# iliasam/STM32F4_SDR_GPS

Hardware: AMD Instinct MI355X
Metric: acquisition hypotheses/sec (PRN x Doppler x phase) (higher is better)
Workload: dtype u1 (MX-FP4 operands, exact f32 accumulation)

## Files before the change

stm32f4_sdr_gps_amd/csrc/gpsx_mx_parts.hpp:

```cpp
#pragma once
#if !defined(GPSX_LAB) && defined(MX_VARIANT_B)
#error "variants of the matrix-core grid kernels for same-box A/B timing build with -DGPSX_LAB only: tools/build_variant.sh"
#endif
#include <cstdlib>

#include "gpsx_anchor_codes.hpp"
#include "gpsx_device.hpp"
#include "gpsx_fold_codes.hpp"
#include "gpsx_kernels.hpp"

namespace gpsx {

namespace {

typedef int v8i __attribute__((ext_vector_type(8)));
typedef int v4i __attribute__((ext_vector_type(4)));
typedef float v16f __attribute__((ext_vector_type(16)));

constexpr int kMxThreads = 512;
constexpr int kMxTiles = 4;
constexpr int kCopyDwords = 260;
constexpr int kVecDwords = 258;
constexpr int kPlaneWordsMx = 66;
constexpr u32 kScaleOne = 0x7F7F7F7Fu;
constexpr u32 kScaleA = 0x72727272u;
constexpr float kAccScale = 1.0f / 8192.0f;
constexpr float kUnscaleSq = 67108864.0f;
constexpr u32 kScaleEight = 0x82828282u;
constexpr u32 kScaleTwo = 0x80808080u;

struct MxShared {
  uint16_t x[1024];
  u32 d[2][514];
  u32 plane[2][16][kPlaneWordsMx];
  u32 base[2][kCopyDwords];
  u32 e8[2][2][8][kCopyDwords];
  u32 corr[2][2][2][128];
  v4i chips_a[16][2][32];
  u32 chip_t[1032];
  u32 ones[2];
  u32 t_lut[768];
  alignas(16) u32 part[8][32][2][32];
};

struct MxFold {
  u32 pair[2][2][1024];
  v4i lut[2][32];
};

__device__ __forceinline__ v8i widen(v4i x) { return v8i{x.x, x.y, x.z, x.w, 0, 0, 0, 0}; }

__device__ __forceinline__ u32 lds_byte(const u32 *words, int byte_index)
{
  return (words[byte_index >> 2] >> ((byte_index & 3) * 8)) & 0xFFu;
}

__device__ __forceinline__ u32 spread8(u32 x)
{
  u32 t = (x | (x << 12)) & 0x000F000Fu;
  t = (t | (t << 6)) & 0x03030303u;
  t = (t | (t << 3)) & 0x11111111u;
  return t;
}

__device__ __forceinline__ int wrap1023(int i)
{
  i = i >= 2 * kChips ? i - 2 * kChips : i;
  return i >= kChips ? i - kChips : i;
}

__device__ __forceinline__ u32 plane_bits9(const u32 *pl, int pos)
{
  return __builtin_amdgcn_alignbit(pl[(pos >> 5) + 1], pl[pos >> 5], (u32)(pos & 31)) & 0x1FFu;
}

struct MxCluster {
  int set, sd, dopp, search;
};
__device__ __forceinline__ MxCluster mx_decode_cluster(int cluster, int n_sets, int n_dopp)
{
  const int set = cluster % n_sets, sd = cluster / n_sets;
  return MxCluster{set, sd, sd % n_dopp, sd / n_dopp};
}
__device__ __forceinline__ u32 mx_step_word(int dopp, int if_hz, int dopp_min_hz, int dopp_step_hz)
{
  const float freq_hz = (float)(if_hz + dopp_min_hz + dopp * dopp_step_hz);
  return nco_step_per_word(freq_hz);
}
__device__ __forceinline__ void mx_load_chips_a(MxShared &sh, const u32 *__restrict__ mx_a, int set, int tid)
{
  const u32 *src_a = mx_a + (size_t)set * (16 * 2 * 32 * 4);
  u32 *dst_a = reinterpret_cast<u32 *>(&sh.chips_a[0][0][0]);
  for (int i = tid; i < 16 * 2 * 32 * 4; i += kMxThreads)
    dst_a[i] = src_a[i];
}
__device__ __forceinline__ void mx_load_tables(MxShared &sh, const u32 *__restrict__ mx_a, const u32 *__restrict__ mx_t, int set, int tid)
{
  mx_load_chips_a(sh, mx_a, set, tid);
  const u32 *src_t = mx_t + (size_t)set * 1032;
  for (int i = tid; i < 1032; i += kMxThreads)
    sh.chip_t[i] = src_t[i];
}

__device__ __forceinline__ void mx_load_block(MxShared &sh, const uint8_t *blk, int if_format, int tid)
{
  for (int i = tid; i < 1024; i += kMxThreads)
    sh.x[i] = i < kWords16 ? load_sign16(blk, i, if_format) : (uint16_t)0;
  if (tid < 2)
    sh.ones[tid] = 0;
}
template <bool WRAP_IN_PLACE = false>
__device__ __forceinline__ void mx_wipe_stream(MxShared &sh, u32 step_word, int tid, int lane)
{
  {
    const u32 *x32 = reinterpret_cast<const u32 *>(sh.x);
    u32 ones_i = 0, ones_q = 0;
    for (int w = tid; w < 514; w += kMxThreads) {
      u32 vi = 0, vq = 0;
      if (w < kWords32) {
        const u32 quad = (step_word * (u32)w) >> 30;
        vi = carrier_i(quad) ^ x32[w];
        vq = carrier_q(quad) ^ x32[w];
      }
      ones_i += __popc(vi);
      ones_q += __popc(vq);
      if (WRAP_IN_PLACE && w == 511) {
        vi = (carrier_i(0u) ^ x32[0]) << 16;
        vq = (carrier_q(0u) ^ x32[0]) << 16;
      }
      sh.d[0][w] = vi;
      sh.d[1][w] = vq;
    }
    ones_i = wave_sum_to_lane63(ones_i);
    ones_q = wave_sum_to_lane63(ones_q);
    if (lane == 63) {
      atomicAdd(&sh.ones[0], ones_i);
      atomicAdd(&sh.ones[1], ones_q);
    }
  }
  if constexpr (!WRAP_IN_PLACE) {
    __syncthreads();
    if (tid < 2)
      sh.d[tid][511] = sh.d[tid][0] << 16;
  }
}
// ... 8 lines not shown
  }
  return v;
}
__device__ void mx_wipe_block(MxShared &sh, u32 step_word, int tid, int lane)
{
  mx_wipe_stream(sh, step_word, tid, lane);
  __syncthreads();
  for (int m = tid; m < 2 * 32 * 16; m += kMxThreads) {
    const int t0 = m & 15, w = (m >> 4) & 31, iq = m >> 9;
    const u32 *src = &sh.d[iq][16 * w];
    u32 bits = 0;
#pragma unroll
    for (int k = 0; k < 16; k++) {
      const u32 sk = src[k];
      bits |= ((sk >> t0) & 1u) << (2 * k);
      bits |= ((sk >> (16 + t0)) & 1u) << (2 * k + 1);
    }
    sh.plane[iq][t0][w] = bits;
  }
  __syncthreads();
  for (int m = tid; m < 2 * 16 * (kPlaneWordsMx - 32); m += kMxThreads) {
    const int w = 32 + m % (kPlaneWordsMx - 32);
    const int r = m / (kPlaneWordsMx - 32);
    sh.plane[r >> 4][r & 15][w] = mx_plane_ext_word(sh.plane[r >> 4][r & 15], w);
  }
}

__device__ __forceinline__ u32 fp4_code(int v)
{
  const u32 m = (u32)(v < 0 ? -v : v);
  return ((0x0765420u >> (4u * (m > 5u ? 5u : m))) & 0xFu) | (v < 0 ? 8u : 0u);
}

__device__ void mx_fill_tables(MxShared &sh, int tid, int nthreads = kMxThreads)
{
  for (int w = tid; w < 512; w += nthreads) {
    const u32 cur = (u32)w & 0xFFu, nxt = ((u32)w >> 1) & 0xFFu;
    const u32 plus = spread8(nxt & ~cur), minus = spread8(cur & ~nxt);
    sh.t_lut[w] = (plus << 2) | (plus << 3) | (minus << 2);
  }
  for (int x = tid; x < 256; x += nthreads)
    sh.t_lut[512 + x] = (spread8((u32)x) << 1) | (spread8(~(u32)x & 0xFFu) * 0xAu);
}

__device__ void mx_vector_phase1(MxShared &sh, int pass, int buf, int tid)
{
  const int t0 = pass - 1;
  for (int m = tid; m < 2 * kVecDwords + 2 * 128; m += kMxThreads) {
    if (m < 2 * kVecDwords) {
      const int iq = m >= kVecDwords, dw = m - iq * kVecDwords;
      u32 packed = 0;
      if (pass < 2) {
        const u32 *dd = sh.d[iq];
#pragma unroll
        for (int e = 0; e < 8; e++) {
          const int k = wrap1023(8 * dw + e);
          const int pos = 16 * k;
          const u32 sum = pop16(__builtin_amdgcn_alignbit(dd[(pos >> 5) + 1], dd[pos >> 5], (u32)(pos & 31)));
          const u32 code = pass == 0 ? (0xFEC0u >> (4u * (sum & 3u))) & 0xFu : (0xEDCA0u >> (4u * (sum >> 2))) & 0xFu;
          packed |= code << (4 * e);
        }
      } else {
        const u32 w = plane_bits9(sh.plane[iq][pass - 2], 8 * dw);
        packed = sh.t_lut[w];
        if (dw == 127 && t0 >= 9) {
          const u32 cur = w & 0xFFu, nxt = (w >> 1) & 0xFFu;
          const int e5 = (int)((nxt >> 5) & 1u) - (int)((cur >> 5) & 1u), e6 = (int)((nxt >> 6) & 1u) - (int)((cur >> 6) & 1u);
// ... 31 lines not shown
{
  for (int m = tid; m < 2 * 256; m += kMxThreads) {
    const int iq = m >> 8, j = m & 255;
    const u32 lo = sh.base[iq][j], hi = sh.base[iq][j + 1];
#pragma unroll
    for (int c = 0; c < 8; c++)
      sh.e8[buf][iq][c][j] = c ? __builtin_amdgcn_alignbit(hi, lo, 4u * (u32)c) : lo;
  }
}

typedef __attribute__((address_space(3))) const u32 lds_cu32;

__device__ __forceinline__ lds_cu32 *lds_opaque(const u32 *p)
{
  u32 a = (u32)(size_t)(lds_cu32 *)p;
  asm volatile("" : "+v"(a));
  return (lds_cu32 *)(size_t)a;
}
__device__ __forceinline__ v4i lds_frag(lds_cu32 *w, int dw)
{
  return v4i{(int)w[dw], (int)w[dw + 1], (int)w[dw + 2], (int)w[dw + 3]};
}

__device__ __forceinline__ u32 mx_patch_wrap(u32 packed, u32 w9, bool patch)
{
  const u32 i5 = 1u + ((w9 >> 6) & 1u) - ((w9 >> 5) & 1u), i6 = 1u + ((w9 >> 7) & 1u) - ((w9 >> 6) & 1u);
  const u32 c5 = (0xDA2u >> (4u * i5)) & 0xFu;
  const u32 c6 = (0xA25u >> (4u * i6)) & 0xFu;
  const u32 patched = (packed & ~0x0FF00000u) | (c5 << 20) | (c6 << 24);
  return patch ? patched : packed;
}

template <bool FOLD = false>
__device__ __forceinline__ void mx_vector_build(MxShared &sh, int p_vec, int tid, MxFold *fold = nullptr)
{
  const int t0 = p_vec - 1, buf = p_vec & 1;
  const bool late = t0 >= 9;
  const int iq = tid >> 8, j = tid & 255, which = (tid >> 7) & 1, dwc = tid & 127;
  const u32 *pl = sh.plane[iq][p_vec - 2];
  const u32 x = __builtin_amdgcn_alignbit(pl[(j >> 2) + 1], pl[j >> 2], 8u * (u32)(j & 3));
  u32 cw = 0, v = 0;
  if constexpr (!FOLD) {
    const int pos = dwc ? 8 * dwc - 1 : 0;
    const u32 y = __builtin_amdgcn_alignbit(pl[(pos >> 5) + 1], pl[pos >> 5], (u32)(pos & 31));
    cw = (dwc ? y : y << 1) & 0x1FFu;
  }
  u32 lo = sh.t_lut[x & 0x1FFu], hi = sh.t_lut[(x >> 8) & 0x1FFu];
  if constexpr (!FOLD)
    v = sh.t_lut[which ? 512u + (cw & 0xFFu) : (late ? cw : 512u + (cw >> 1))];
  if (late) {
    lo = mx_patch_wrap(lo, x & 0x1FFu, j == 127);
    hi = mx_patch_wrap(hi, (x >> 8) & 0x1FFu, j == 126);
    if constexpr (!FOLD) {
      if (which == 0)
        v ^= (v & 0x44444444u) << 1;
      if (dwc == 0)
        v = (v & ~0xFu) | (which ? 0u : ((cw & 2u) ? 0x2u : 0xAu));
    }
  }
  if constexpr (!FOLD) {
    v &= dwc == 127 ? 0x0FFFFFFFu : 0xFFFFFFFFu;
    if ((which && !late) || t0 == 8)
      v = 0;
    sh.corr[buf][iq][which][dwc] = v;
  } else {
    const int pos = 4 * j + kChips - 2;
    const u32 z = __builtin_amdgcn_alignbit(pl[(pos >> 5) + 1], pl[pos >> 5], (u32)(pos & 31)) & 31u;
    v4i pr = fold->lut[late][z];
    if (late && j == 0) {
      pr.x = (int)(gpsx_fold_pair(true, 0, (int)(z & 1u), (int)((z >> 1) & 1u)) << kGpsxFoldShift);
      pr.y = (int)(gpsx_fold_pair(true, 1, (int)((z >> 1) & 1u), (int)((z >> 2) & 1u)) << kGpsxFoldShift);
    }
    *reinterpret_cast<v4i *>(&fold->pair[buf][iq][4 * j]) = pr;
  }
  u32 *dst = &sh.e8[buf][iq][0][j];
#pragma unroll
  for (int c = 0; c < 8; c++)
    dst[c * kCopyDwords] = c ? __builtin_amdgcn_alignbit(hi, lo, 4u * (u32)c) : lo;
}

struct MxFoldRegs {
  lds_cu32 *w;
  u32 mask, pi, pq;
};
template <int S, int NT, u32 SCALE_A = kScaleA, bool FOLD = false>
__device__ __forceinline__ void mx_pass_step(lds_cu32 *wi, lds_cu32 *wq, const v4i *ca, v4i (&a)[16], v4i &fi, v4i &fq,
                                             v16f (&acc)[2][NT], u32 scale_b, MxFoldRegs *fold = nullptr)
{
  constexpr int kSteps = 16 + NT - 1;
  constexpr bool more = S + 1 < kSteps;
  constexpr bool pair_next = FOLD && more && S + 1 >= 15, patched = FOLD && S >= 15;
  v4i fi_next = fi, fq_next = fq;
  u32 pi_next = 0, pq_next = 0;
  if constexpr (more) {
    fi_next = lds_frag(wi, 8 * (S + 1));
    fq_next = lds_frag(wq, 8 * (S + 1));
    if constexpr (S + 1 < 16)
      a[S + 1] = ca[(S + 1) * 64];
    if constexpr (pair_next) {
      pi_next = fold->w[64 * (S + 1 - 15)];
      pq_next = fold->w[64 * (S + 1 - 15) + 1024];
    }
  }
  constexpr int j_lo = S - 15 > 0 ? S - 15 : 0, j_hi = S < NT - 1 ? S : NT - 1;
#pragma unroll
  for (int j = j_lo + (patched ? 1 : 0); j <= j_hi; j++) {
    acc[0][j] = __builtin_amdgcn_mfma_scale_f32_32x32x64_f8f6f4(widen(a[S - j]), widen(fi), acc[0][j], 4, 4, 0, SCALE_A, 0, scale_b);
    acc[1][j] = __builtin_amdgcn_mfma_scale_f32_32x32x64_f8f6f4(widen(a[S - j]), widen(fq), acc[1][j], 4, 4, 0, SCALE_A, 0, scale_b);
  }
  if constexpr (patched) {
    fi.w = (int)((fold->mask & fold->pi) | (~fold->mask & (u32)fi.w));
    fq.w = (int)((fold->mask & fold->pq) | (~fold->mask & (u32)fq.w));
    acc[0][j_lo] = __builtin_amdgcn_mfma_scale_f32_32x32x64_f8f6f4(widen(a[15]), widen(fi), acc[0][j_lo], 4, 4, 0, SCALE_A, 0, scale_b);
    acc[1][j_lo] = __builtin_amdgcn_mfma_scale_f32_32x32x64_f8f6f4(widen(a[15]), widen(fq), acc[1][j_lo], 4, 4, 0, SCALE_A, 0, scale_b);
  }
  if constexpr (more) {
    __builtin_amdgcn_sched_group_barrier(0x100, (S + 1 < 16 ? 5 : 4) + (pair_next ? 2 : 0), 0);
    if constexpr (patched) {
      __builtin_amdgcn_sched_group_barrier(0x008, 2 * (j_hi - j_lo), 0);
      __builtin_amdgcn_sched_group_barrier(0x002, 2, 0);
      __builtin_amdgcn_sched_group_barrier(0x008, 2, 0);
    } else {
      __builtin_amdgcn_sched_group_barrier(0x008, 2 * (j_hi - j_lo + 1), 0);
    }
  }
  __builtin_amdgcn_sched_barrier(0);
  fi = fi_next;
  fq = fq_next;
  if constexpr (FOLD) {
    fold->pi = pi_next;
    fold->pq = pq_next;
  }
  if constexpr (more)
    mx_pass_step<S + 1, NT, SCALE_A, FOLD>(wi, wq, ca, a, fi, fq, acc, scale_b, fold);
}

template <int S, int NT>
__device__ __forceinline__ void mx_pass_step_inplace(lds_cu32 *wi, lds_cu32 *wq, const v4i *ca, v4i (&a)[16], v4i &fi, v4i &fq,
                                                     v16f (&acc)[2][NT], u32 scale_b)
{
  constexpr int kSteps = 16 + NT - 1;
  constexpr bool more = S + 1 < kSteps;
  if constexpr (more && S + 1 < 16)
    a[S + 1] = ca[(S + 1) * 64];
  constexpr int j_lo = S - 15 > 0 ? S - 15 : 0, j_hi = S < NT - 1 ? S : NT - 1;
#pragma unroll
  for (int j = j_lo; j <= j_hi; j++)
    acc[0][j] = __builtin_amdgcn_mfma_scale_f32_32x32x64_f8f6f4(widen(a[S - j]), widen(fi), acc[0][j], 4, 4, 0, kScaleA, 0, scale_b);
  if constexpr (more)
    fi = lds_frag(wi, 8 * (S + 1));
#pragma unroll
  for (int j = j_lo; j <= j_hi; j++)
    acc[1][j] = __builtin_amdgcn_mfma_scale_f32_32x32x64_f8f6f4(widen(a[S - j]), widen(fq), acc[1][j], 4, 4, 0, kScaleA, 0, scale_b);
  if constexpr (more)
    fq = lds_frag(wq, 8 * (S + 1));
  if constexpr (more) {
    if constexpr (S + 1 < 16)
      __builtin_amdgcn_sched_group_barrier(0x100, 1, 0);
    __builtin_amdgcn_sched_group_barrier(0x008, j_hi - j_lo + 1, 0);
    __builtin_amdgcn_sched_group_barrier(0x100, 2, 0);
    __builtin_amdgcn_sched_group_barrier(0x008, j_hi - j_lo + 1, 0);
    __builtin_amdgcn_sched_group_barrier(0x100, 2, 0);
  }
  __builtin_amdgcn_sched_barrier(0);
  if constexpr (more)
    mx_pass_step_inplace<S + 1, NT>(wi, wq, ca, a, fi, fq, acc, scale_b);
}

template <bool AHEAD, int NT, u32 SCALE_A = kScaleA, bool FOLD = false>
__device__ __forceinline__ void mx_pass(const MxShared &sh, int buf, int lane, int q0_tile, v16f (&acc)[2][NT],
                                        u32 scale_b, v4i a_corr, bool with_corr, const u32 *fold_pair = nullptr)
{
  static_assert(!FOLD || (AHEAD && NT == kMxTiles), "the fold is the single-block form's");
  const int n = lane & 31, h = lane >> 5;
  const u32 *e8 = &sh.e8[buf][0][0][0];
  lds_cu32 *wi = lds_opaque(e8 + (n & 7) * kCopyDwords + 4 * (q0_tile + h) + (n >> 3));
  lds_cu32 *wq = lds_opaque(e8 + (8 + (n & 7)) * kCopyDwords + 4 * (q0_tile + h) + (n >> 3));
  const v4i *ca = &sh.chips_a[0][h][n];
  v4i a[16];
  if constexpr (AHEAD) {
    v4i fi = lds_frag(wi, 0), fq = lds_frag(wq, 0);
    a[0] = ca[0];
    if constexpr (FOLD) {
      MxFoldRegs fold{lds_opaque(fold_pair + 32 * q0_tile + n), h && with_corr ? kGpsxFoldMask : 0u, 0u, 0u};
      mx_pass_step<0, NT, SCALE_A, true>(wi, wq, ca, a, fi, fq, acc, scale_b, &fold);
    } else {
      mx_pass_step<0, NT, SCALE_A>(wi, wq, ca, a, fi, fq, acc, scale_b);
    }
  } else {
    static_assert(SCALE_A == kScaleA, "the in-place walk is the sign-only grid's");
    v4i fi = lds_frag(wi, 0), fq = lds_frag(wq, 0);
    a[0] = ca[0];
    mx_pass_step_inplace<0, NT>(wi, wq, ca, a, fi, fq, acc, scale_b);
  }
  if (!FOLD && with_corr) {
    lds_cu32 *cw = lds_opaque(&sh.corr[buf][0][h][4 * q0_tile + (n >> 3)]);
#pragma unroll
    for (int j = 0; j < NT; j++) {
      const v4i gi = v4i{(int)(cw[8 * j] >> (4 * (n & 7))), 0, 0, 0};
      const v4i gq = v4i{(int)(cw[8 * j + 2 * 128] >> (4 * (n & 7))), 0, 0, 0};
      acc[0][j] = __builtin_amdgcn_mfma_scale_f32_32x32x64_f8f6f4(widen(a_corr), widen(gi), acc[0][j], 4, 4, 0, kScaleA, 0,
                                                                   kScaleOne);
      acc[1][j] = __builtin_amdgcn_mfma_scale_f32_32x32x64_f8f6f4(widen(a_corr), widen(gq), acc[1][j], 4, 4, 0, kScaleA, 0,
// ... 239 lines not shown
```

stm32f4_sdr_gps_amd/csrc/k_acq_mx.hip:

```cpp
#include "gpsx_mx_parts.hpp"

namespace gpsx {

__global__ void k_build_mx_tables(const u32 *__restrict__ chipbits, int n_slots, u32 *__restrict__ mx_a, u32 *__restrict__ mx_t)
{
  const int n_sets = (n_slots + 31) / 32;
  const int idx = blockIdx.x * blockDim.x + threadIdx.x;
  const int per_set = 16 * 2 * 32 * 4 + 1032;
  if (idx >= n_sets * per_set)
    return;
  const int set = idx / per_set, r = idx - set * per_set;
  if (r < 16 * 2 * 32 * 4) {
    const int dw = r & 3, p = (r >> 2) & 31, h = (r >> 7) & 1, kappa = r >> 8;
    const int slot = 32 * set + p;
    const u32 word = slot < n_slots ? chipbits[(size_t)slot * 32 + 2 * kappa + h] : 0u;
    mx_a[(size_t)set * (16 * 2 * 32 * 4) + r] = spread8((word >> (8 * dw)) & 0xFFu) << 1;
  } else {
    const int c = r - 16 * 2 * 32 * 4 - 1;
    u32 w = 0;
    if (c >= 0 && c < kChips)
      for (int p = 0; p < 32; p++) {
        const int slot = 32 * set + p;
        if (slot < n_slots)
          w |= ((chipbits[(size_t)slot * 32 + (c >> 5)] >> (c & 31)) & 1u) << p;
      }
    mx_t[(size_t)set * 1032 + (c + 1)] = w;
  }
}

void launch_build_mx_tables(hipStream_t s, const uint32_t *d_chipbits, int n_slots, uint32_t *d_mx_a, uint32_t *d_mx_t)
{
  const int n_sets = (n_slots + 31) / 32;
  const int n = n_sets * (16 * 2 * 32 * 4 + 1032);
  hipLaunchKernelGGL(k_build_mx_tables, dim3((n + 255) / 256), dim3(256), 0, s, d_chipbits, n_slots, d_mx_a, d_mx_t);
}

namespace {

constexpr int kMxNoSet = -1;
constexpr int kPasses = 17;
constexpr int kPassesAnchor = 16;
constexpr int kAnchorDwords = 392;

__device__ __forceinline__ void mx_planes_half(MxShared &sh, int t0_lo, int v, int lane)
{
  const int iq = v >> 1, t0_first = t0_lo + 4 * (v & 1);
  const int t0 = t0_first + (lane & 3), rot = lane >> 2;
#pragma unroll 1
  for (int it = 0; it < 2; it++) {
    const int w = rot + 16 * it;
    const u32 *src = &sh.d[iq][16 * w];
    u32 bits = 0;
#pragma unroll
    for (int k = 0; k < 16; k++) {
      const int kk = (k + rot) & 15;
      const u32 sk = src[kk];
      bits |= ((sk >> t0) & 1u) << (2 * kk);
      bits |= ((sk >> (16 + t0)) & 1u) << (2 * kk + 1);
    }
    sh.plane[iq][t0][w] = bits;
  }
  __builtin_amdgcn_fence(__ATOMIC_ACQ_REL, "wavefront");
  asm volatile("s_waitcnt lgkmcnt(0)" ::: "memory");
#pragma unroll 1
  for (int m = lane; m < 4 * (kPlaneWordsMx - 32); m += 64) {
    const int r = m / (kPlaneWordsMx - 32), w = 32 + m % (kPlaneWordsMx - 32);
    u32 *pl = sh.plane[iq][t0_first + r];
    pl[w] = mx_plane_ext_word(pl, w);
  }
}

__device__ __forceinline__ void mx_anchor_build(MxShared &sh, u32 *dst, int tid)
{
  const int iq = tid >> 8, j = tid & 255;
  const u32 *dd = sh.d[iq];
  u64 bits = 0;
#pragma unroll
  for (int e = 0; e < 8; e++) {
    const int pos = 16 * wrap1023(8 * j + e);
    const u32 sum = pop16(__builtin_amdgcn_alignbit(dd[(pos >> 5) + 1], dd[pos >> 5], (u32)(pos & 31)));
    bits |= (u64)gpsx_anchor_code((int)sum) << (6 * e);
  }
  const u32 lo = (u32)bits, hi = (u32)(bits >> 32);
  const u32 lo_pair = dpp<0xB1>(lo, lo);
  u32 *d3 = dst + iq * kAnchorDwords + 3 * (j >> 1);
  if (j & 1) {
    d3[2] = (lo >> 16) | (hi << 16);
  } else {
    d3[0] = lo;
    d3[1] = hi | (lo_pair << 16);
  }
}

struct AnchorRaw {
  u32 d[7];
};
__device__ __forceinline__ AnchorRaw mx_anchor_raw(lds_cu32 *w, int dw)
{
  AnchorRaw r;
#pragma unroll
  for (int i = 0; i < 7; i++)
    r.d[i] = w[dw + i];
  return r;
}
__device__ __forceinline__ v8i mx_anchor_frag(const AnchorRaw &r, u32 shift)
{
  v8i f = {0, 0, 0, 0, 0, 0, 0, 0};
#pragma unroll
  for (int i = 0; i < 6; i++)
    f[i] = (int)__builtin_amdgcn_alignbit(r.d[i + 1], r.d[i], shift);
  return f;
}
template <int S, int NT>
__device__ __forceinline__ void mx_anchor_step(lds_cu32 *wi, lds_cu32 *wq, const v4i *ca, v4i (&a)[16], v8i &fi, v8i &fq,
                                               v16f (&acc)[2][NT], u32 shift)
{
  constexpr int kSteps = 16 + NT - 1;
  constexpr bool more = S + 1 < kSteps;
  AnchorRaw ri, rq;
  if constexpr (more) {
    ri = mx_anchor_raw(wi, 12 * (S + 1));
    rq = mx_anchor_raw(wq, 12 * (S + 1));
    if constexpr (S + 1 < 16)
      a[S + 1] = ca[(S + 1) * 64];
  }
  constexpr int j_lo = S - 15 > 0 ? S - 15 : 0, j_hi = S < NT - 1 ? S : NT - 1;
#pragma unroll
  for (int j = j_lo; j <= j_hi; j++) {
    acc[0][j] = __builtin_amdgcn_mfma_scale_f32_32x32x64_f8f6f4(widen(a[S - j]), fi, acc[0][j], 4, 3, 0, kScaleA, 0, kScaleTwo);
    acc[1][j] = __builtin_amdgcn_mfma_scale_f32_32x32x64_f8f6f4(widen(a[S - j]), fq, acc[1][j], 4, 3, 0, kScaleA, 0, kScaleTwo);
  }
  if constexpr (more) {
    __builtin_amdgcn_sched_group_barrier(0x100, S + 1 < 16 ? 9 : 8, 0);
    __builtin_amdgcn_sched_group_barrier(0x008, 2 * (j_hi - j_lo + 1), 0);
  }
  __builtin_amdgcn_sched_barrier(0);
  if constexpr (more) {
    fi = mx_anchor_frag(ri, shift);
    fq = mx_anchor_frag(rq, shift);
    __builtin_amdgcn_sched_barrier(0);
    mx_anchor_step<S + 1, NT>(wi, wq, ca, a, fi, fq, acc, shift);
  }
}
template <int NT>
__device__ __forceinline__ void mx_anchor_pass(const MxShared &sh, const u32 *anchor, int lane, int q0_tile, v16f (&acc)[2][NT])
{
  const int n = lane & 31, h = lane >> 5;
  const u32 shift = (u32)(6 * n) & 31u;
  lds_cu32 *wi = lds_opaque(anchor + 6 * (q0_tile + h) + ((6 * n) >> 5));
  lds_cu32 *wq = lds_opaque(anchor + kAnchorDwords + 6 * (q0_tile + h) + ((6 * n) >> 5));
  const v4i *ca = &sh.chips_a[0][h][n];
  v4i a[16];
  v8i fi = mx_anchor_frag(mx_anchor_raw(wi, 0), shift), fq = mx_anchor_frag(mx_anchor_raw(wq, 0), shift);
  a[0] = ca[0];
  mx_anchor_step<0, NT>(wi, wq, ca, a, fi, fq, acc, shift);
}

__device__ __forceinline__ void mx_vector_build_direct(MxShared &sh, int which, int t0s, u32 *e8_dst, int tid)
{
  const int iq = tid >> 8, j = tid & 255;
  const u32 *dd = sh.d[iq];
  u32 w2[2] = {0, 0};
#pragma unroll
  for (int e = 0; e < 16; e++) {
    const int k = wrap1023(8 * j + e);
    const int pos = 16 * k + t0s;
    const u32 sum = pop16(__builtin_amdgcn_alignbit(dd[(pos >> 5) + 1], dd[pos >> 5], (u32)(pos & 31)));
    const u32 code = which == 0 ? (0xFEC0u >> (4u * (sum & 3u))) & 0xFu : (0xEDCA0u >> (4u * (sum >> 2))) & 0xFu;
    w2[e >> 3] |= code << (4 * (e & 7));
  }
  u32 *dst = e8_dst + (iq * 8) * kCopyDwords + j;
#pragma unroll
  for (int c = 0; c < 8; c++)
    dst[c * kCopyDwords] = c ? __builtin_amdgcn_alignbit(w2[1], w2[0], 4u * (u32)c) : w2[0];
}

__device__ __forceinline__ void mx_direct_terms(const MxShared &sh, int lane, int q0_tile, v16f (&acc)[2][kMxTiles], int t0s,
                                                int win_start, int win_stop)
// ... 252 lines not shown
  if (SEARCH && !DIRECT) {
#pragma unroll
    for (int r = 0; r < 16; r++) {
      const int p_off = ((r & 3) + 8 * (r >> 2)) * 64;
      atomicMax(slot + p_off, best[DIRECT ? 0 : r]);
      atomicAdd(slot + p_off + 32, total[DIRECT ? 0 : r]);
    }
  }
}

__device__ __forceinline__ void mx_epilogue_store(int lane, int q0_tile, int t0, const v16f (&acc)[2][kMxTiles], u32 group_mask,
                                                  uint16_t *__restrict__ plane0, size_t prn_stride, int slot0, int n_prn)
{
  const int n = lane & 31, h = lane >> 5;
#pragma unroll
  for (int j = 0; j < kMxTiles; j++) {
    const int q = 32 * (q0_tile + 2 * j) + n;
    uint16_t *v = plane0 + (size_t)t0 * 1024 + (size_t)(q & 3) * 256 + (size_t)(q >> 2);
#pragma unroll
    for (int g = 0; g < 4; g++) {
#pragma unroll
      for (int rr = 0; rr < 4; rr++) {
        const int r = 4 * g + rr;
        const int p = (r & 3) + 8 * (r >> 2) + 4 * h;
        const u32 val = mag8_f32(acc[0][j][r], acc[1][j][r]);
        if (((group_mask >> g) & 1u) && slot0 + p < n_prn)
          v[(size_t)p * prn_stride] = (uint16_t)val;
      }
      __builtin_amdgcn_sched_barrier(0);
    }
  }
}

struct MxSingleShared {
  MxShared mx;
  MxFold fold;
};
__device__ __forceinline__ void mx_fill_fold_lut(MxFold &fold, int t)
{
  if (t < 64) {
    const int late = t >> 5, z = t & 31;
    v4i e;
#pragma unroll
    for (int i = 0; i < 4; i++)
      e[i] = (int)(gpsx_fold_pair(late != 0, 2, (z >> i) & 1, (z >> (i + 1)) & 1) << kGpsxFoldShift);
    fold.lut[late][z] = e;
  }
}

__device__ __forceinline__ void mx_single(MxShared &sh, MxFold &fold, const AcqParams &prm, int cluster_lo,
                                          const uint8_t *__restrict__ if_blocks, const u32 *__restrict__ mx_a,
                                          const u32 *__restrict__ mx_t, gpsx_peak_t *__restrict__ peaks)
{
  const int tid = threadIdx.x;
  const int lane = tid & 63, wave = __builtin_amdgcn_readfirstlane(tid >> 6);
  const int role = wave >> 2;
  const int q0_tile = 8 * (wave >> 1) + (wave & 1);

  const int n_sets = (prm.n_groups + 3) / 4;
  const MxCluster c = mx_decode_cluster(cluster_lo + (int)blockIdx.x, n_sets, prm.n_dopp);
  const int set = c.set, sd = c.sd, dopp = c.dopp, search = c.search;
  u32 group_mask = 0;
#pragma unroll
  for (int g = 0; g < 4; g++) {
    const int group = 4 * set + g;
    const int unit = sd * prm.n_groups + group;
    if (group < prm.n_groups && unit >= prm.unit_lo && unit < prm.unit_hi)
      group_mask |= 1u << g;
  }
  group_mask = (u32)__builtin_amdgcn_readfirstlane((int)group_mask);
  if (group_mask == 0)
    return;
  const u32 step_word = mx_step_word(dopp, prm.if_hz, prm.dopp_min_hz, prm.dopp_step_hz);

  if (set != kMxNoSet) {
    mx_load_tables(sh, mx_a, mx_t, set, tid);
  }
  for (int i = tid; i < 8 * 32 * 2 * 32 / 4; i += kMxThreads)
    reinterpret_cast<uint4 *>(&sh.part[0][0][0][0])[i] = make_uint4(0, 0, 0, 0);
  const size_t block_bytes = prm.if_format == GPSX_IF_2BIT_SM ? GPSX_BYTES_PER_MS_2BIT : kBytes;
  const uint8_t *block0 = if_blocks + (size_t)(search * prm.search_stride_blocks) * block_bytes;
  mx_load_block(sh, block0, prm.if_format, tid);

  __syncthreads();
  u32 kq[kMxTiles];
#pragma unroll
  for (int j = 0; j < kMxTiles; j++) {
    kq[j] = (u32)(2047 - 2 * (32 * (q0_tile + 2 * j) + (lane & 31)));
    asm volatile("" : "+v"(kq[j]));
  }
  const int n_pass = kPassesAnchor;
#pragma unroll 1
  for (int once = 0; once < 1; once++) {
    mx_wipe_stream<true>(sh, step_word, tid, lane);
    __syncthreads();
    mx_anchor_build(sh, &sh.e8[0][0][0][0], tid);

    v16f acc[2][kMxTiles];
    if (role == 0)
      mx_init_acc(sh.ones, lane, q0_tile, acc, prm.win_start, prm.win_stop, kGpsxAnchorPassBias);

    auto opaque = [](int v) {
      asm volatile("" : "+v"(v));
      return v;
    };
    __syncthreads();
    if (role) {
      mx_planes_half(sh, 0, wave & 3, opaque(lane));
      mx_fill_tables(sh, opaque(tid) & 255, 256);
      mx_fill_fold_lut(fold, opaque(tid) & 255);
      mx_planes_half(sh, 8, wave & 3, opaque(lane));
      mx_init_acc(sh.ones, opaque(lane), q0_tile, acc, prm.win_start, prm.win_stop, kGpsxAnchorPassBias);
    }
    mx_anchor_pass(sh, &sh.e8[0][0][0][0], lane, q0_tile, acc);
    if (!role)
      mx_epilogue_single(sh, lane, kq, 0, acc);
    __syncthreads();
    mx_vector_build<true>(sh, 2, opaque(tid), &fold);
#pragma unroll 1
    for (int hs = 2; hs <= 2 * n_pass; hs++) {
      if ((hs & 1) == 0) {
        __syncthreads();
        const int p_vec = (hs >> 1) + 1;
        if (p_vec < n_pass)
          mx_vector_build<true>(sh, p_vec + 1, tid, &fold);
      }
      const int x = hs - role;
      const bool active = x >= 0 && x < 2 * n_pass;
      const int p = (x >> 1) + 1;
      if (active && (x & 1) == 0) {
        mx_pass<true, kMxTiles, kScaleA, true>(sh, p & 1, lane, q0_tile, acc, p == 1 ? kScaleEight : kScaleOne, v4i{0, 0, 0, 0},
                                               p >= 2 && p != 9, &fold.pair[p & 1][0][0]);
        if (p == 9)
          mx_half_switch(sh, lane, q0_tile, acc, prm.win_start, prm.win_stop);
      }
      if (active && (x & 1) && p >= 1)
        mx_epilogue_single(sh, lane, kq, p - 1, acc);
    }
  }
  __syncthreads();
  {
    const int which = tid >> 8, p = (tid >> 3) & 31, b = tid & 7;
    const int slot = 32 * set + p;
    const u32 *row = sh.part[b][p][which];
    u32 vals[32];
#pragma unroll
    for (int l = 0; l < 32; l++)
      vals[l] = row[(l + tid) & 31];
    u32 k = 0, t = 0;
#pragma unroll
    for (int l = 0; l < 32; l++) {
      k = vals[l] > k ? vals[l] : k;
      t += vals[l];
    }
    if (((group_mask >> (p >> 3)) & 1u) && slot < prm.n_prn && b < prm.n_bits) {
      const size_t idx = ((size_t)(search * prm.n_prn + slot) * prm.n_dopp + dopp) * prm.n_bits + b;
      uint2 *pk = reinterpret_cast<uint2 *>(&peaks[idx]);
      if (which == 0) {
        const u32 max_val = k >> 11;
        pk[0] = make_uint2(max_val, max_val ? 2047u - (k & 2047u) : 0u);
      } else {
        pk[1] = make_uint2(t, t / (2u * kChips));
      }
    }
    if (prm.keys && which == 0) {
      unsigned long long key = 0;
      if (b < prm.n_bits) {
        const u32 max_val = k >> 11, phase = max_val ? 2047u - (k & 2047u) : 0u;
        key = ((unsigned long long)max_val << 14) | (unsigned long long)(16383u - (8u * phase + (u32)b));
      }
      key = mx_max8_u64(key);
      if (b == 0 && ((group_mask >> (p >> 3)) & 1u) && slot < prm.n_prn)
        prm.keys[(size_t)(search * prm.n_prn + slot) * prm.n_dopp + dopp] = (int64_t)key;
    }
  }
}

template <int MODE>
__device__ __forceinline__ void mx_unit(MxShared &sh, const AcqParams &prm, int cluster_lo,
                                        const uint8_t *__restrict__ if_blocks, const u32 *__restrict__ mx_a,
                                        const u32 *__restrict__ mx_t, gpsx_peak_t *__restrict__ peaks, u32 *__restrict__ energy,
                                        u32 *__restrict__ flags)
{
  constexpr bool MULTI = MODE == kMxWalk || MODE == kMxWalk16, STORE = MODE == kMxStore, S16 = MODE == kMxWalk16;
  constexpr bool SPLIT = MODE == kMxSplit;
  typedef SumRecT<S16> SumRec;
  const int wg = (int)blockIdx.x;
// ... 184 lines not shown
        if (which == 0)
          atomicMax(&energy[idx], k);
        else
          atomicAdd(&energy[n_planes + idx], t);
      } else if (which == 0) {
        const u32 max_val = k >> 11;
        pk[0] = make_uint2(max_val, max_val ? 2047u - (k & 2047u) : 0u);
      } else {
        pk[1] = make_uint2(t, t / (2u * kChips));
      }
    }
    if constexpr (!SPLIT) {
      if (prm.keys && which == 0) {
        unsigned long long key = 0;
        if (b < prm.n_bits) {
          const u32 max_val = k >> 11, phase = max_val ? 2047u - (k & 2047u) : 0u;
          key = ((unsigned long long)max_val << 14) | (unsigned long long)(16383u - (8u * phase + (u32)b));
        }
        key = mx_max8_u64(key);
        if (b == 0 && ((group_mask >> (p >> 3)) & 1u) && slot < prm.n_prn)
          prm.keys[(size_t)(search * prm.n_prn + slot) * prm.n_dopp + dopp] = (int64_t)key;
      }
    }
  }
}

}

template <int MODE>
__global__ __launch_bounds__(kMxThreads, 1) void k_acq_mx(GPSX_K_ACQ_MX_PARAMS)
{
  if constexpr (MODE == kMxSingle) {
    __shared__ MxSingleShared sh;
    mx_single(sh.mx, sh.fold, prm, cluster_lo, if_blocks, mx_a, mx_t, peaks);
  } else {
    __shared__ MxShared sh;
    mx_unit<MODE>(sh, prm, cluster_lo, if_blocks, mx_a, mx_t, peaks, energy, flags);
  }
}

void launch_acq_mx(hipStream_t s, const AcqPlan &p, const AcqParams &prm, const uint8_t *d_if, const uint32_t *d_mx_a,
                   const uint32_t *d_mx_t, uint32_t *d_planes, uint32_t *d_energy)
{
  if (p.c_hi <= p.c_lo)
    return;
  const dim3 grid((unsigned)p.grid), block(kMxThreads);
  gpsx_peak_t *d_peaks = prm.peaks;
  switch (p.form) {
  case AcqForm::kMxStore:
    hipLaunchKernelGGL(k_acq_mx<kMxStore>, grid, block, 0, s, prm, p.c_lo, d_if, d_mx_a, d_mx_t, d_peaks, d_energy, (u32 *)nullptr);
    launch_acq_vals_search(s, prm, reinterpret_cast<const uint16_t *>(d_energy), d_peaks, p.n_peaks);
    break;
  case AcqForm::kMxWalk: {
    u32 *d_flags = d_energy + acq_mx_energy_bytes(p.grid) / sizeof(u32) - p.grid;
    (void)hipMemsetAsync(d_flags - kMxZeroRecBytes / sizeof(u32), 0, kMxZeroRecBytes, s);
    hipLaunchKernelGGL(k_acq_mx<kMxWalk16>, grid, block, 0, s, prm, p.c_lo, d_if, d_mx_a, d_mx_t, d_peaks, d_energy, d_flags);
    if (p.walk24)
      hipLaunchKernelGGL(k_acq_mx<kMxWalk>, grid, block, 0, s, prm, p.c_lo, d_if, d_mx_a, d_mx_t, d_peaks, d_energy, d_flags);
    break;
  }
  case AcqForm::kMxByte:
    launch_acq_mx_byte(s, (unsigned)p.grid, prm, p.c_lo, d_if, d_mx_a, d_mx_t);
    break;
  case AcqForm::kMxSplit:
    hipLaunchKernelGGL(k_acq_mx<kMxSplit>, grid, block, 0, s, prm, p.c_lo, d_if, d_mx_a, d_mx_t, d_peaks, d_planes, (u32 *)nullptr);
    launch_acq_finalize(s, d_planes, d_planes + p.n_peaks, p.n_peaks, d_peaks, prm.keys);
    break;
// ... 14 lines not shown
```

Before: 1396 billion.

## Transpose MFMA operands in single-block path and reduce peaks in-register

The single-block acquisition path swaps the A/B operands of the scaled MFMA so each lane holds a code-phase row layout instead of a PRN-column layout. The epilogue then reduces max and sum keys across its registers and writes them with LDS atomics into a much smaller partial buffer, replacing the large per-lane partial table and its 32-way final scan. The half-switch correction now reads a precomputed float2 LDS table built during setup. The aim is to cut epilogue LDS traffic and the shared-memory footprint, at the cost of atomics and extra setup work.

Result: faster. 1515 billion, median of 6 (+8.6%).

```diff
diff --git a/stm32f4_sdr_gps_amd/csrc/gpsx_mx_parts.hpp b/stm32f4_sdr_gps_amd/csrc/gpsx_mx_parts.hpp
--- a/stm32f4_sdr_gps_amd/csrc/gpsx_mx_parts.hpp
+++ b/stm32f4_sdr_gps_amd/csrc/gpsx_mx_parts.hpp
@@ -29,7 +29,7 @@
 constexpr u32 kScaleEight = 0x82828282u;
 constexpr u32 kScaleTwo = 0x80808080u;
 
-struct MxShared {
+struct MxSharedCore {
   uint16_t x[1024];
   u32 d[2][514];
   u32 plane[2][16][kPlaneWordsMx];
@@ -40,6 +40,8 @@
   u32 chip_t[1032];
   u32 ones[2];
   u32 t_lut[768];
+};
+struct MxShared : MxSharedCore {
   alignas(16) u32 part[8][32][2][32];
 };
 
@@ -87,14 +89,14 @@
   const float freq_hz = (float)(if_hz + dopp_min_hz + dopp * dopp_step_hz);
   return nco_step_per_word(freq_hz);
 }
-__device__ __forceinline__ void mx_load_chips_a(MxShared &sh, const u32 *__restrict__ mx_a, int set, int tid)
+__device__ __forceinline__ void mx_load_chips_a(MxSharedCore &sh, const u32 *__restrict__ mx_a, int set, int tid)
 {
   const u32 *src_a = mx_a + (size_t)set * (16 * 2 * 32 * 4);
   u32 *dst_a = reinterpret_cast<u32 *>(&sh.chips_a[0][0][0]);
   for (int i = tid; i < 16 * 2 * 32 * 4; i += kMxThreads)
     dst_a[i] = src_a[i];
 }
-__device__ __forceinline__ void mx_load_tables(MxShared &sh, const u32 *__restrict__ mx_a, const u32 *__restrict__ mx_t, int set, int tid)
+__device__ __forceinline__ void mx_load_tables(MxSharedCore &sh, const u32 *__restrict__ mx_a, const u32 *__restrict__ mx_t, int set, int tid)
 {
   mx_load_chips_a(sh, mx_a, set, tid);
   const u32 *src_t = mx_t + (size_t)set * 1032;
@@ -102,7 +104,7 @@
     sh.chip_t[i] = src_t[i];
 }
 
-__device__ __forceinline__ void mx_load_block(MxShared &sh, const uint8_t *blk, int if_format, int tid)
+__device__ __forceinline__ void mx_load_block(MxSharedCore &sh, const uint8_t *blk, int if_format, int tid)
 {
   for (int i = tid; i < 1024; i += kMxThreads)
     sh.x[i] = i < kWords16 ? load_sign16(blk, i, if_format) : (uint16_t)0;
@@ -110,7 +112,7 @@
     sh.ones[tid] = 0;
 }
 template <bool WRAP_IN_PLACE = false>
-__device__ __forceinline__ void mx_wipe_stream(MxShared &sh, u32 step_word, int tid, int lane)
+__device__ __forceinline__ void mx_wipe_stream(MxSharedCore &sh, u32 step_word, int tid, int lane)
 {
   {
     const u32 *x32 = reinterpret_cast<const u32 *>(sh.x);
@@ -185,7 +187,7 @@
   return ((0x0765420u >> (4u * (m > 5u ? 5u : m))) & 0xFu) | (v < 0 ? 8u : 0u);
 }
 
-__device__ void mx_fill_tables(MxShared &sh, int tid, int nthreads = kMxThreads)
+__device__ void mx_fill_tables(MxSharedCore &sh, int tid, int nthreads = kMxThreads)
 {
   for (int w = tid; w < 512; w += nthreads) {
     const u32 cur = (u32)w & 0xFFu, nxt = ((u32)w >> 1) & 0xFFu;
@@ -283,7 +285,7 @@
 }
 
 template <bool FOLD = false>
-__device__ __forceinline__ void mx_vector_build(MxShared &sh, int p_vec, int tid, MxFold *fold = nullptr)
+__device__ __forceinline__ void mx_vector_build(MxSharedCore &sh, int p_vec, int tid, MxFold *fold = nullptr)
 {
   const int t0 = p_vec - 1, buf = p_vec & 1;
   const bool late = t0 >= 9;
@@ -334,6 +336,14 @@
   lds_cu32 *w;
   u32 mask, pi, pq;
 };
+template <bool TR, u32 SCALE_C>
+__device__ __forceinline__ v16f mx_mfma(v4i chips, v4i frag, v16f acc, u32 scale_f)
+{
+  if constexpr (TR)
+    return __builtin_amdgcn_mfma_scale_f32_32x32x64_f8f6f4(widen(frag), widen(chips), acc, 4, 4, 0, scale_f, 0, SCALE_C);
+  else
+    return __builtin_amdgcn_mfma_scale_f32_32x32x64_f8f6f4(widen(chips), widen(frag), acc, 4, 4, 0, SCALE_C, 0, scale_f);
+}
 template <int S, int NT, u32 SCALE_A = kScaleA, bool FOLD = false>
 __device__ __forceinline__ void mx_pass_step(lds_cu32 *wi, lds_cu32 *wq, const v4i *ca, v4i (&a)[16], v4i &fi, v4i &fq,
                                              v16f (&acc)[2][NT], u32 scale_b, MxFoldRegs *fold = nullptr)
@@ -356,14 +366,14 @@
   constexpr int j_lo = S - 15 > 0 ? S - 15 : 0, j_hi = S < NT - 1 ? S : NT - 1;
 #pragma unroll
   for (int j = j_lo + (patched ? 1 : 0); j <= j_hi; j++) {
-    acc[0][j] = __builtin_amdgcn_mfma_scale_f32_32x32x64_f8f6f4(widen(a[S - j]), widen(fi), acc[0][j], 4, 4, 0, SCALE_A, 0, scale_b);
-    acc[1][j] = __builtin_amdgcn_mfma_scale_f32_32x32x64_f8f6f4(widen(a[S - j]), widen(fq), acc[1][j], 4, 4, 0, SCALE_A, 0, scale_b);
+    acc[0][j] = mx_mfma<FOLD, SCALE_A>(a[S - j], fi, acc[0][j], scale_b);
+    acc[1][j] = mx_mfma<FOLD, SCALE_A>(a[S - j], fq, acc[1][j], scale_b);
   }
   if constexpr (patched) {
     fi.w = (int)((fold->mask & fold->pi) | (~fold->mask & (u32)fi.w));
     fq.w = (int)((fold->mask & fold->pq) | (~fold->mask & (u32)fq.w));
-    acc[0][j_lo] = __builtin_amdgcn_mfma_scale_f32_32x32x64_f8f6f4(widen(a[15]), widen(fi), acc[0][j_lo], 4, 4, 0, SCALE_A, 0, scale_b);
-    acc[1][j_lo] = __builtin_amdgcn_mfma_scale_f32_32x32x64_f8f6f4(widen(a[15]), widen(fq), acc[1][j_lo], 4, 4, 0, SCALE_A, 0, scale_b);
+    acc[0][j_lo] = mx_mfma<FOLD, SCALE_A>(a[15], fi, acc[0][j_lo], scale_b);
+    acc[1][j_lo] = mx_mfma<FOLD, SCALE_A>(a[15], fq, acc[1][j_lo], scale_b);
   }
   if constexpr (more) {
     __builtin_amdgcn_sched_group_barrier(0x100, (S + 1 < 16 ? 5 : 4) + (pair_next ? 2 : 0), 0);
@@ -419,7 +429,7 @@
 }
 
 template <bool AHEAD, int NT, u32 SCALE_A = kScaleA, bool FOLD = false>
-__device__ __forceinline__ void mx_pass(const MxShared &sh, int buf, int lane, int q0_tile, v16f (&acc)[2][NT],
+__device__ __forceinline__ void mx_pass(const MxSharedCore &sh, int buf, int lane, int q0_tile, v16f (&acc)[2][NT],
                                         u32 scale_b, v4i a_corr, bool with_corr, const u32 *fold_pair = nullptr)
 {
   static_assert(!FOLD || (AHEAD && NT == kMxTiles), "the fold is the single-block form's");
diff --git a/stm32f4_sdr_gps_amd/csrc/gpsx_mx_transposed.hpp b/stm32f4_sdr_gps_amd/csrc/gpsx_mx_transposed.hpp
--- /dev/null
+++ b/stm32f4_sdr_gps_amd/csrc/gpsx_mx_transposed.hpp
@@ -0,0 +1,24 @@
+#pragma once
+#include <stdint.h>
+
+constexpr int kGpsxMxtLocals = 64;
+constexpr int kGpsxMxtKeyShift = 6;
+constexpr int kGpsxKeyShift = 11;
+
+constexpr int gpsx_mxt_q0_tile(int wave) { return 8 * (wave >> 1) + (wave & 1); }
+constexpr int gpsx_mxt_row(int h, int r) { return (r & 3) + 8 * (r >> 2) + 4 * h; }
+constexpr int gpsx_mxt_q(int wave, int h, int j, int r) { return 32 * (gpsx_mxt_q0_tile(wave) + 2 * j) + gpsx_mxt_row(h, r); }
+constexpr int gpsx_mxt_local(int j, int r) { return 16 * j + r; }
+constexpr uint32_t gpsx_mxt_code(int j, int r) { return (uint32_t)(kGpsxMxtLocals - 1 - gpsx_mxt_local(j, r)); }
+constexpr uint32_t gpsx_mxt_local_key(uint32_t bits, int j, int r) { return (bits << kGpsxMxtKeyShift) | gpsx_mxt_code(j, r); }
+constexpr int gpsx_mxt_q_of_local(int q_first, int local)
+{
+  return q_first + ((local & 48) << 2) + ((local & 12) << 1) + (local & 3);
+}
+constexpr uint32_t gpsx_mxt_global_key(uint32_t local_key, int q_first, int half)
+{
+  const int local = (int)((local_key & (kGpsxMxtLocals - 1)) ^ (kGpsxMxtLocals - 1));
+  const int q = gpsx_mxt_q_of_local(q_first, local);
+  return ((local_key >> kGpsxMxtKeyShift) << kGpsxKeyShift) | (uint32_t)(2047 - (2 * q + half));
+}
+constexpr int gpsx_mxt_group(int lane) { return (lane & 31) >> 3; }
diff --git a/stm32f4_sdr_gps_amd/csrc/k_acq_mx.hip b/stm32f4_sdr_gps_amd/csrc/k_acq_mx.hip
--- a/stm32f4_sdr_gps_amd/csrc/k_acq_mx.hip
+++ b/stm32f4_sdr_gps_amd/csrc/k_acq_mx.hip
@@ -1,4 +1,5 @@
 #include "gpsx_mx_parts.hpp"
+#include "gpsx_mx_transposed.hpp"
 
 namespace gpsx {
 
@@ -42,7 +43,7 @@
 constexpr int kPassesAnchor = 16;
 constexpr int kAnchorDwords = 392;
 
-__device__ __forceinline__ void mx_planes_half(MxShared &sh, int t0_lo, int v, int lane)
+__device__ __forceinline__ void mx_planes_half(MxSharedCore &sh, int t0_lo, int v, int lane)
 {
   const int iq = v >> 1, t0_first = t0_lo + 4 * (v & 1);
   const int t0 = t0_first + (lane & 3), rot = lane >> 2;
@@ -70,7 +71,7 @@
   }
 }
 
-__device__ __forceinline__ void mx_anchor_build(MxShared &sh, u32 *dst, int tid)
+__device__ __forceinline__ void mx_anchor_build(MxSharedCore &sh, u32 *dst, int tid)
 {
   const int iq = tid >> 8, j = tid & 255;
   const u32 *dd = sh.d[iq];
@@ -127,8 +128,8 @@
   constexpr int j_lo = S - 15 > 0 ? S - 15 : 0, j_hi = S < NT - 1 ? S : NT - 1;
 #pragma unroll
   for (int j = j_lo; j <= j_hi; j++) {
-    acc[0][j] = __builtin_amdgcn_mfma_scale_f32_32x32x64_f8f6f4(widen(a[S - j]), fi, acc[0][j], 4, 3, 0, kScaleA, 0, kScaleTwo);
-    acc[1][j] = __builtin_amdgcn_mfma_scale_f32_32x32x64_f8f6f4(widen(a[S - j]), fq, acc[1][j], 4, 3, 0, kScaleA, 0, kScaleTwo);
+    acc[0][j] = __builtin_amdgcn_mfma_scale_f32_32x32x64_f8f6f4(fi, widen(a[S - j]), acc[0][j], 3, 4, 0, kScaleTwo, 0, kScaleA);
+    acc[1][j] = __builtin_amdgcn_mfma_scale_f32_32x32x64_f8f6f4(fq, widen(a[S - j]), acc[1][j], 3, 4, 0, kScaleTwo, 0, kScaleA);
   }
   if constexpr (more) {
     __builtin_amdgcn_sched_group_barrier(0x100, S + 1 < 16 ? 9 : 8, 0);
@@ -143,7 +144,7 @@
   }
 }
 template <int NT>
-__device__ __forceinline__ void mx_anchor_pass(const MxShared &sh, const u32 *anchor, int lane, int q0_tile, v16f (&acc)[2][NT])
+__device__ __forceinline__ void mx_anchor_pass(const MxSharedCore &sh, const u32 *anchor, int lane, int q0_tile, v16f (&acc)[2][NT])
 {
   const int n = lane & 31, h = lane >> 5;
   const u32 shift = (u32)(6 * n) & 31u;
@@ -462,10 +463,195 @@
   }
 }
 
+constexpr int kHsStride = 1026;
 struct MxSingleShared {
-  MxShared mx;
+  MxSharedCore mx;
   MxFold fold;
+  alignas(16) u32 part[8][2][2][32];
+  alignas(16) float2 hs[2][kHsStride];
 };
+
+struct MxtWindow {
+  int lo0, hi0, lo1, hi1;
+};
+__device__ __forceinline__ MxtWindow mxt_window(int win_start, int win_stop)
+{
+  MxtWindow w;
+  w.lo0 = (win_start + 1) >> 1;
+  w.hi0 = min(kChips, (win_stop + 1) >> 1);
+  w.lo1 = win_start >> 1;
+  w.hi1 = min(kChips, win_stop >> 1);
+  return w;
+}
+__device__ __forceinline__ bool mxt_wave_whole(int q0_tile, int win_start, int win_stop)
+{
+  const MxtWindow w = mxt_window(win_start, win_stop);
+  const int q_lo = 32 * q0_tile, q_hi = 32 * (q0_tile + 2 * (kMxTiles - 1)) + 31;
+  return q_lo >= w.lo0 && q_hi < w.hi1;
+}
+
+__device__ __forceinline__ void mxt_init_acc(const u32 *ones, int lane, int q0_tile, v16f (&acc)[2][kMxTiles], int win_start,
+                                             int win_stop, int pass_bias)
+{
+  const float base_i = (float)((int)ones[0] + 8192 - kHalf - pass_bias) * kAccScale,
+              base_q = (float)((int)ones[1] + 8192 - kHalf - pass_bias) * kAccScale;
+  if (mxt_wave_whole(q0_tile, win_start, win_stop)) {
+#pragma unroll
+    for (int j = 0; j < kMxTiles; j++)
+#pragma unroll
+      for (int r = 0; r < 16; r++) {
+        acc[0][j][r] = base_i;
+        acc[1][j][r] = base_q;
+      }
+  } else {
+    const MxtWindow w = mxt_window(win_start, win_stop);
+    const int h = lane >> 5;
+    const u32 span = (u32)max(w.hi0 - w.lo0, 0);
+#pragma unroll
+    for (int j = 0; j < kMxTiles; j++)
+#pragma unroll
+      for (int r = 0; r < 16; r++) {
+        const int q = 32 * (q0_tile + 2 * j) + gpsx_mxt_row(h, r);
+        const bool in_win = (u32)(q - w.lo0) < span;
+        acc[0][j][r] = in_win ? base_i : base_i + kOutside;
+        acc[1][j][r] = in_win ? base_q : base_q + kOutside;
+      }
+  }
+}
+
+__device__ __forceinline__ void mxt_half_switch_build(const MxSharedCore &sh, float2 (*hs)[kHsStride], int t, int n)
+{
+  const int popw[2] = {(int)__popc(sh.d[0][0] & 0xFFu), (int)__popc(sh.d[1][0] & 0xFFu)};
+#pragma unroll 1
+  for (int m = t; m < 512; m += n) {
+    float row[2][2][2];
+#pragma unroll
+    for (int s = 0; s < 2; s++) {
+      const u32 w = sh.d[s][m], before = sh.d[s][m > 0 ? m - 1 : 0] >> 24;
+#pragma unroll
+      for (int k = 0; k < 2; k++) {
+        const u32 cur = (w >> (16 * k)) & 0xFFu;
+        int fa = -(2 * (int)__popc(cur & 0x7Fu) - 7);
+        int fk = -popw[s];
+        if (2 * m + k > 0) {
+          const u32 prev = (k ? (w >> 8) & 0xFFu : before) | (cur << 8);
+          fk -= (int)__popc(prev);
+          fa -= 16 - 2 * (int)__popc(prev);
+        }
+        row[0][k][s] = (float)fk * kAccScale;
+        row[1][k][s] = (float)(fk + fa) * kAccScale;
+      }
+    }
+#pragma unroll
+    for (int c = 0; c < 2; c++)
+      *reinterpret_cast<float4 *>(&hs[c][2 * m]) = make_float4(row[c][0][0], row[c][0][1], row[c][1][0], row[c][1][1]);
+  }
+}
+
+__device__ __forceinline__ void mxt_half_switch(const MxSharedCore &sh, const float2 (*hs)[kHsStride], int lane, int q0_tile,
+                                                v16f (&acc)[2][kMxTiles], int win_start, int win_stop)
+{
+  asm volatile("" : "+v"(lane));
+  const int prn = lane & 31, h = lane >> 5;
+  const u32 wrap_i = (sh.d[0][0] & 0xFFu) << 8, wrap_q = (sh.d[1][0] & 0xFFu) << 8;
+  const float nbeta_i = -(float)(16 - 2 * (int)__popc(wrap_i)) * kAccScale, nbeta_q = -(float)(16 - 2 * (int)__popc(wrap_q)) * kAccScale;
+  const int q4_first = 32 * q0_tile + 4 * h, q4_last = q4_first + 64 * (kMxTiles - 1) + 24;
+  const float2 *tab = &hs[(sh.chip_t[1022 + 1] >> prn) & 1u][q4_first];
+  const u32 *cw = &sh.chip_t[kChips - 3 - q4_last];
+#pragma unroll
+  for (int j = 0; j < kMxTiles; j++) {
+#pragma unroll
+    for (int g = 0; g < 4; g++) {
+      const int dq = 64 * j + 8 * g;
+      const float4 t01 = *reinterpret_cast<const float4 *>(&tab[dq]), t23 = *reinterpret_cast<const float4 *>(&tab[dq + 2]);
+      const uint4 w = *reinterpret_cast<const uint4 *>(&cw[64 * (kMxTiles - 1) + 24 - dq]);
+      const float ti[4] = {t01.x, t01.z, t23.x, t23.z}, tq[4] = {t01.y, t01.w, t23.y, t23.w};
+      const u32 wi[4] = {w.w, w.z, w.y, w.x};
+#pragma unroll
+      for (int i = 0; i < 4; i++) {
+        const float c1 = (float)((wi[i] >> prn) & 1u);
+        acc[0][j][4 * g + i] += __builtin_fmaf(c1, nbeta_i, ti[i]);
+        acc[1][j][4 * g + i] += __builtin_fmaf(c1, nbeta_q, tq[i]);
+      }
+    }
+  }
+  if (!mxt_wave_whole(q0_tile, win_start, win_stop)) {
+    const MxtWindow w = mxt_window(win_start, win_stop);
+    const bool any = win_start < win_stop;
+    const int q_in = any && w.lo1 != w.lo0 ? w.lo1 : -1, q_out = any && w.hi1 != w.hi0 ? w.hi1 : -1;
+#pragma unroll
+    for (int j = 0; j < kMxTiles; j++) {
+      const int tile = q0_tile + 2 * j;
+      if ((q_in >> 5) != tile && (q_out >> 5) != tile)
+        continue;
+#pragma unroll
+      for (int r = 0; r < 16; r++) {
+        const int q = 32 * tile + gpsx_mxt_row(h, r);
+        const float edge = (q == q_in ? -kOutside : 0.0f) + (q == q_out ? kOutside : 0.0f);
+        acc[0][j][r] += edge;
+        acc[1][j][r] += edge;
+      }
+    }
+  }
+}
+
+__device__ __forceinline__ void mxt_epilogue(u32 *part, int lane, int q0_tile, int t0, const v16f (&acc)[2][kMxTiles])
+{
+  const int b = t0 & 7, half = t0 >> 3;
+  u32 best[4], total[4];
+#pragma unroll
+  for (int c = 0; c < 4; c++) {
+    best[c] = 0;
+    total[c] = c ? 0u : 0u - (u32)kGpsxMxtLocals * kRootBias;
+  }
+  mx_round_toward_zero();
+#pragma unroll
+  for (int jp = 0; jp < kMxTiles; jp += 2) {
+#pragma unroll
+    for (int r0 = 0; r0 < 16; r0 += 4) {
+      float ev[8];
+      u32 e_max = 0;
+#pragma unroll
+      for (int i = 0; i < 8; i++) {
+        ev[i] = clip_square_sum(acc[0][jp + (i >> 2)][r0 + (i & 3)], acc[1][jp + (i >> 2)][r0 + (i & 3)]);
+        e_max = max(e_max, __float_as_uint(ev[i]));
+      }
+      const bool small = __builtin_amdgcn_ballot_w64(e_max >= 0x3C800000u ) == 0;
+      u32 bits[8];
+      if (__builtin_expect(small, 1)) {
+#pragma unroll
+        for (int i = 0; i < 8; i++)
+          bits[i] = root_bits_small(ev[i]);
+      } else {
+        float ci[8], cq[8];
+#pragma unroll
+        for (int i = 0; i < 8; i++) {
+          ci[i] = acc[0][jp + (i >> 2)][r0 + (i & 3)];
+          cq[i] = acc[1][jp + (i >> 2)][r0 + (i & 3)];
+        }
+        mx_roots_exact<8>(ci, cq, bits);
+#pragma unroll
+        for (int i = 0; i < 8; i++)
+          bits[i] += kRootBias;
+      }
+#pragma unroll
+      for (int rr = 0; rr < 4; rr++) {
+        const u32 k0 = gpsx_mxt_local_key(bits[rr], jp, r0 + rr), k1 = gpsx_mxt_local_key(bits[4 + rr], jp + 1, r0 + rr);
+        best[rr] = max(max(best[rr], k0), k1);
+        total[rr] = total[rr] + bits[rr] + bits[4 + rr];
+      }
+#pragma unroll
+      for (int rr = 0; rr < 4; rr++)
+        asm volatile("" : "+v"(best[rr]), "+v"(total[rr]));
+      __builtin_amdgcn_sched_barrier(0);
+    }
+  }
+  mx_round_to_nearest();
+  const u32 key = gpsx_mxt_global_key(max(max(best[0], best[1]), max(best[2], best[3])), 32 * q0_tile + 4 * (lane >> 5), half);
+  u32 *slot = part + (2 * b) * 64 + lane;
+  atomicMax(slot, key);
+  atomicAdd(slot + 64, total[0] + total[1] + total[2] + total[3]);
+}
 __device__ __forceinline__ void mx_fill_fold_lut(MxFold &fold, int t)
 {
   if (t < 64) {
@@ -478,10 +664,13 @@
   }
 }
 
-__device__ __forceinline__ void mx_single(MxShared &sh, MxFold &fold, const AcqParams &prm, int cluster_lo,
+__device__ __forceinline__ void mx_single(MxSingleShared &shs, const AcqParams &prm, int cluster_lo,
                                           const uint8_t *__restrict__ if_blocks, const u32 *__restrict__ mx_a,
                                           const u32 *__restrict__ mx_t, gpsx_peak_t *__restrict__ peaks)
 {
+  MxSharedCore &sh = shs.mx;
+  MxFold &fold = shs.fold;
+  u32 *part = &shs.part[0][0][0][0];
   const int tid = threadIdx.x;
   const int lane = tid & 63, wave = __builtin_amdgcn_readfirstlane(tid >> 6);
   const int role = wave >> 2;
@@ -506,19 +695,13 @@
   if (set != kMxNoSet) {
     mx_load_tables(sh, mx_a, mx_t, set, tid);
   }
-  for (int i = tid; i < 8 * 32 * 2 * 32 / 4; i += kMxThreads)
-    reinterpret_cast<uint4 *>(&sh.part[0][0][0][0])[i] = make_uint4(0, 0, 0, 0);
+  if (tid < (int)(sizeof(shs.part) / sizeof(uint4)))
+    reinterpret_cast<uint4 *>(part)[tid] = make_uint4(0, 0, 0, 0);
   const size_t block_bytes = prm.if_format == GPSX_IF_2BIT_SM ? GPSX_BYTES_PER_MS_2BIT : kBytes;
   const uint8_t *block0 = if_blocks + (size_t)(search * prm.search_stride_blocks) * block_bytes;
   mx_load_block(sh, block0, prm.if_format, tid);
 
   __syncthreads();
-  u32 kq[kMxTiles];
-#pragma unroll
-  for (int j = 0; j < kMxTiles; j++) {
-    kq[j] = (u32)(2047 - 2 * (32 * (q0_tile + 2 * j) + (lane & 31)));
-    asm volatile("" : "+v"(kq[j]));
-  }
   const int n_pass = kPassesAnchor;
 #pragma unroll 1
   for (int once = 0; once < 1; once++) {
@@ -528,7 +711,7 @@
 
     v16f acc[2][kMxTiles];
     if (role == 0)
-      mx_init_acc(sh.ones, lane, q0_tile, acc, prm.win_start, prm.win_stop, kGpsxAnchorPassBias);
+      mxt_init_acc(sh.ones, lane, q0_tile, acc, prm.win_start, prm.win_stop, kGpsxAnchorPassBias);
 
     auto opaque = [](int v) {
       asm volatile("" : "+v"(v));
@@ -540,11 +723,12 @@
       mx_fill_tables(sh, opaque(tid) & 255, 256);
       mx_fill_fold_lut(fold, opaque(tid) & 255);
       mx_planes_half(sh, 8, wave & 3, opaque(lane));
-      mx_init_acc(sh.ones, opaque(lane), q0_tile, acc, prm.win_start, prm.win_stop, kGpsxAnchorPassBias);
+      mxt_half_switch_build(sh, shs.hs, opaque(tid) & 255, 256);
+      mxt_init_acc(sh.ones, opaque(lane), q0_tile, acc, prm.win_start, prm.win_stop, kGpsxAnchorPassBias);
     }
     mx_anchor_pass(sh, &sh.e8[0][0][0][0], lane, q0_tile, acc);
     if (!role)
-      mx_epilogue_single(sh, lane, kq, 0, acc);
+      mxt_epilogue(part, lane, q0_tile, 0, acc);
     __syncthreads();
     mx_vector_build<true>(sh, 2, opaque(tid), &fold);
 #pragma unroll 1
@@ -562,27 +746,18 @@
         mx_pass<true, kMxTiles, kScaleA, true>(sh, p & 1, lane, q0_tile, acc, p == 1 ? kScaleEight : kScaleOne, v4i{0, 0, 0, 0},
                                                p >= 2 && p != 9, &fold.pair[p & 1][0][0]);
         if (p == 9)
-          mx_half_switch(sh, lane, q0_tile, acc, prm.win_start, prm.win_stop);
+          mxt_half_switch(sh, shs.hs, lane, q0_tile, acc, prm.win_start, prm.win_stop);
       }
       if (active && (x & 1) && p >= 1)
-        mx_epilogue_single(sh, lane, kq, p - 1, acc);
+        mxt_epilogue(part, lane, q0_tile, p - 1, acc);
     }
   }
   __syncthreads();
   {
     const int which = tid >> 8, p = (tid >> 3) & 31, b = tid & 7;
     const int slot = 32 * set + p;
-    const u32 *row = sh.part[b][p][which];
-    u32 vals[32];
-#pragma unroll
-    for (int l = 0; l < 32; l++)
-      vals[l] = row[(l + tid) & 31];
-    u32 k = 0, t = 0;
-#pragma unroll
-    for (int l = 0; l < 32; l++) {
-      k = vals[l] > k ? vals[l] : k;
-      t += vals[l];
-    }
+    const u32 v0 = shs.part[b][which][0][p], v1 = shs.part[b][which][1][p];
+    const u32 k = v0 > v1 ? v0 : v1, t = v0 + v1;
     if (((group_mask >> (p >> 3)) & 1u) && slot < prm.n_prn && b < prm.n_bits) {
       const size_t idx = ((size_t)(search * prm.n_prn + slot) * prm.n_dopp + dopp) * prm.n_bits + b;
       uint2 *pk = reinterpret_cast<uint2 *>(&peaks[idx]);
@@ -833,7 +1008,7 @@
 {
   if constexpr (MODE == kMxSingle) {
     __shared__ MxSingleShared sh;
-    mx_single(sh.mx, sh.fold, prm, cluster_lo, if_blocks, mx_a, mx_t, peaks);
+    mx_single(sh, prm, cluster_lo, if_blocks, mx_a, mx_t, peaks);
   } else {
     __shared__ MxShared sh;
     mx_unit<MODE>(sh, prm, cluster_lo, if_blocks, mx_a, mx_t, peaks, energy, flags);
```
